# simochen/flowtrack.pytorch

Measured on AMD Instinct MI355X. Metric: pose crops/sec (ResNet-50 + 3-deconv head, 256x192), higher is better.
Workload: dtype fp16; 1 GPU; ResNet-50 pose head fp16, batch 64 x 256x192 synthetic crops per GPU (BASELINE.json configs[1]); per_gpu_batch=64, resident_batches=4, parallelism=dp1: batch sharded, one process per GPU

## Files before the change

flowtrack/pytorch_amd/csrc/conv_common.h:

```cpp
#pragma once
#include <stdlib.h>

#include <type_traits>

#include "ft_common.h"

#define FT_LDS_BARRIER() asm volatile("s_barrier" ::: "memory")

namespace ft {

struct ConvParams {
  const char* x;
  const char* w;
  const float* scale;
  const float* shift;
  const char* res;
  char* y;
  int M;
  int HqWq, Wq;
  int Hi, Wi;
  int sy;
  int x_cstride, x_coff;
  int kh, kw;
  int dmul;
// ... 229 lines not shown
        }
        return;
      }
      half_t* ybase = reinterpret_cast<half_t*>(p.y) + p.y_coff + co0;
      for (int idx = tid; idx < BP * NCH; idx += NT) {
        const int pl = idx / NCH, ch = idx % NCH;
        const long long o = s_opix[pl];
        if (o >= 0 && co0 + ch * 8 < p.Cout) {
          const uint4_t v = *reinterpret_cast<const uint4_t*>(s_tile + pl * ROWB + ((ch ^ (pl & (NCH - 1))) << 4));
          store_out16(ybase + o * p.y_cstride + ch * 8, v);
        }
      }
      return;
    }
  }

#pragma unroll
  for (int j = 0; j < MT_P; ++j) {
    const int m = m0 + wp * WT_P + j * 32 + l31;
    if (m >= p.M) continue;
    const int n = m / p.HqWq;
    const int rem = m - n * p.HqWq;
    const int qy = rem / p.Wq;
    const int qx = rem - qy * p.Wq;
    const int oy = qy * p.omul + py, ox = qx * p.omul + px;
    const size_t opix = ((size_t)n * p.Ho + oy) * p.Wo + ox;
#pragma unroll
    for (int i = 0; i < MT_C; ++i) {
#pragma unroll
      for (int rg = 0; rg < 4; ++rg) {
        const int cb = co0 + wc * WT_C + i * 32 + 8 * rg + 4 * lhi;
        if (cb >= p.Cout) continue;
        float v[4];
#pragma unroll
        for (int e = 0; e < 4; ++e) v[e] = acc[i][j][rg * 4 + e];
        if (p.scale) {
          const float4_t s = *reinterpret_cast<const float4_t*>(p.scale + cb);
#pragma unroll
          for (int e = 0; e < 4; ++e) v[e] *= s[e];
        }
        if (p.shift) {
          const float4_t s = *reinterpret_cast<const float4_t*>(p.shift + cb);
#pragma unroll
          for (int e = 0; e < 4; ++e) v[e] += s[e];
        }
        const bool full = cb + 3 < p.Cout;
        if (p.res) {
          const T* rp = reinterpret_cast<const T*>(p.res) + opix * p.res_cstride + p.res_coff + cb;
          if (full) {
            float r4[4];
            load4(rp, r4);
#pragma unroll
            for (int e = 0; e < 4; ++e) v[e] += r4[e];
          } else {
#pragma unroll
            for (int e = 0; e < 4; ++e)
              if (cb + e < p.Cout) v[e] += (float)rp[e];
          }
        }
#pragma unroll
        for (int e = 0; e < 4; ++e) v[e] = apply_act(v[e], p.act, p.slope);
        if (p.out_layout == FT_LAYOUT_NHWC) {
          T* yp = reinterpret_cast<T*>(p.y) + opix * p.y_cstride + p.y_coff + cb;
          if (full) {
            store4(yp, v);
          } else {
#pragma unroll
            for (int e = 0; e < 4; ++e)
              if (cb + e < p.Cout) yp[e] = (T)v[e];
          }
        } else {
          float* yp = reinterpret_cast<float*>(p.y);
          const size_t hw = (size_t)p.Ho * p.Wo;
          const size_t pix = (size_t)oy * p.Wo + ox;
#pragma unroll
          for (int e = 0; e < 4; ++e)
            if (cb + e < p.Cout) yp[((size_t)n * p.Cout + cb + e) * hw + pix] = v[e];
        }
      }
    }
  }
}

int launch_igemm8(const ConvParams& p, unsigned tiles, hipStream_t s);

}
```

flowtrack/pytorch_amd/csrc/conv_igemm.hip:

```cpp
#include <stdlib.h>

#include <type_traits>

#include "ft_common.h"

#ifndef FT_DMA_BKB
#define FT_DMA_BKB 64
#endif
#ifndef FT_DMA_STAGES
#define FT_DMA_STAGES 3
#endif
#include "conv_common.h"

namespace ft {

template <typename T, int BP, int BC, int WGP, int WGC, int BKB>
__global__ __launch_bounds__(256) void conv_igemm_kernel(const ConvParams p) {
  constexpr int VEC = Elem<T>::VEC;
  constexpr int CH = BKB / 16;
  constexpr int RPP = 256 / CH;
  constexpr int NB = BP / RPP;
  constexpr int NA = (BC + RPP - 1) / RPP;
  constexpr int WT_P = BP / WGP, WT_C = BC / WGC;
  constexpr int MT_P = WT_P / 32, MT_C = WT_C / 32;
// ... 2232 lines not shown
  p.h_ty = ceil_div(Hq, th);
  p.h_tx = ceil_div(Wq, tw);
  p.h_pw = tw + kq - 1;
  p.h_npix = (th + kq - 1) * p.h_pw;
  const int cch = d->transposed ? 64 : FT_HALO_CCH;
  p.h_npww = ceil_div(ceil_div(p.h_npix, 1024 / (cch * 2)), 4);
  if (p.h_npww > (d->transposed ? 5 : 6)) return FT_ERR_UNSUPPORTED;
  p.h_pb = p.h_npww * 4 * 1024;
  const int S = d->transposed ? 4 : 3;
  const size_t lds = (size_t)S * bc * 64 + 2 * (size_t)p.h_pb + 1024 + 128 * 8;
  const int N = p.M / p.HqWq;
  p.npt = N * p.h_ty * p.h_tx;
  p.nct = g.cout_pad / bc;
  if ((long long)p.npt * p.nct * p.nph > 0x7fffffffLL) return FT_ERR_UNSUPPORTED;
  dim3 grid(p.npt * p.nct * p.nph);
  int rc;
  if (d->transposed) {
    if (bc == 128) rc = tw == 16 ? launch_halo_k<128, 16, 4, 2, 4, 64>(p, grid, lds, s) : launch_halo_k<128, 8, 4, 2, 4, 64>(p, grid, lds, s);
    else rc = tw == 16 ? launch_halo_k<64, 16, 4, 2, 4, 64>(p, grid, lds, s) : launch_halo_k<64, 8, 4, 2, 4, 64>(p, grid, lds, s);
  } else {
    if (bc == 128) rc = tw == 16 ? launch_halo_k<128, 16, 9, 3, 3, FT_HALO_CCH>(p, grid, lds, s) : launch_halo_k<128, 8, 9, 3, 3, FT_HALO_CCH>(p, grid, lds, s);
    else rc = tw == 16 ? launch_halo_k<64, 16, 9, 3, 3, FT_HALO_CCH>(p, grid, lds, s) : launch_halo_k<64, 8, 9, 3, 3, FT_HALO_CCH>(p, grid, lds, s);
  }
  if (rc != FT_OK) return rc;
  FT_LAUNCH_CHECK("conv_halo_kernel");
  return FT_OK;
}

constexpr int kHintHalo = 1 << 30;

static bool stem_ok(const ft_conv_desc* d, const Geometry& g) {
  if (!g.rowpack || d->dtype != FT_F16 || d->has_residual || d->Cout != 64 || d->x_coff != 0) return false;
  if (!((d->kh == 7 && d->stride == 2) || (d->kh == 3 && d->stride == 1))) return false;
  const int runb = g.cin_pad * 2;
  if (!(runb == 64 || runb == 128 || (runb == 256 && d->kh == 7))) return false;
  if ((d->stride * d->x_cstride * 2) % 16 != 0 || d->pad - d->x_lpad > 0) return false;
  return d->out_layout == FT_LAYOUT_NHWC && d->y_coff % 8 == 0 && d->y_cstride % 8 == 0;
}

static bool halo_ok(const ft_conv_desc* d, const Geometry& g) {
  if (g.rowpack) return stem_ok(d, g);
  if (!g.dma || d->dtype != FT_F16 || d->has_residual) return false;
  if (!(d->transposed || (d->kh == 3 && d->kw == 3 && d->stride == 1 && d->pad == 1))) return false;
  return d->out_layout == FT_LAYOUT_NHWC && d->Cout % 8 == 0 && d->y_coff % 8 == 0 && d->y_cstride % 8 == 0;
}

static bool shift_n_ok(const ft_conv_desc* d, const Geometry& g) {
  if (d->shift_nstride < d->Cout || d->shift_nstride % 4 || d->pool || d->tail_cout > 0 || d->x2_cin > 0 || d->kh != 7 || d->stride != 2)
    return false;
  if (!stem_ok(d, g)) return false;
  if ((unsigned long long)d->N * d->Hi * d->x_wpitch * d->x_cstride * 2 >= (1ull << 31)) return false;
  int pw, npww, ntiles;
  size_t lds;
  return stem_persist_plan(d, g, &pw, &npww, &lds, &ntiles);
}

extern "C" int ft_conv_shift_nstride_supported(const ft_conv_desc* d) {
  Geometry g;
  const int st = geometry(d, &g);
  if (st != FT_OK) return st;
  return shift_n_ok(d, g) ? FT_OK : FT_ERR_UNSUPPORTED;
}

constexpr int kHintSkShift = 21;
__host__ __device__ constexpr int hint_sk(int code) { return code < 4 ? 1 << code : (code == 4 ? 3 : code + 0); }
constexpr int sk_code(int sk) { return sk == 1 ? 0 : sk == 2 ? 1 : sk == 4 ? 2 : sk == 8 ? 3 : sk == 3 ? 4 : sk; }

constexpr int kWide8 = 3;

static bool igemm8_ok(const ft_conv_desc* d, const Geometry& g) {
  if (!(g.dma && !g.rowpack && d->dtype == FT_F16 && g.kc2 == 0 && g.kc % 2 == 0 && g.cout_pad % 256 == 0 && g.nk / 2 >= 2)) return false;
  if (d->has_residual) return false;
  if ((unsigned long long)g.nphases * g.cout_pad * g.kpad * 2 >= (1ull << 31)) return false;
  if (g.cout_pad > 1024) return false;
  if (d->tail_cout > 0) return d->Cout == 256 && d->tail_cout <= 24;
  if (!(d->out_layout == FT_LAYOUT_NHWC && d->Cout % 8 == 0 && d->y_coff % 8 == 0 && d->y_cstride % 8 == 0)) return false;
  return (unsigned long long)d->N * d->Ho * d->Wo * d->y_cstride * 2 < (1ull << 31);
}

static bool tile_valid(const ft_conv_desc* d, const Geometry& g, int bp, int bc, int ks, int wide = 0, bool halo = false,
                       int sk = 1) {
  if (!g.dma) return false;
  if (wide == kWide8) {
    if (!igemm8_ok(d, g) || bp != 256 || bc != 256 || ks != 1 || halo) return false;
    if (sk != 1) {
      const int nk8 = g.nk / 2, per = (nk8 + sk - 1) / sk;
      if (sk < 2 || sk > 8 || d->tail_cout > 0 || per < 4 || nk8 - (sk - 1) * per < 2) return false;
    }
    return true;
  }
  if (sk != 1) {
    if (!(sk == 2 || sk == 4 || sk == 8) || ks != 1 || halo || g.kc2 > 0 || d->tail_cout > 0 || g.rowpack || bp > 128) return false;
    if ((g.nk >> wide) / sk < 4) return false;
  }
  if (g.kc2 > 0) {
    if (ks != 1 || halo) return false;
    if (wide && (g.kc2 % 2 != 0 || (g.kc >> 1) < 2)) return false;
  }
  if (halo) return halo_ok(d, g) && bp == 128 && (bc == 64 || (bc == 128 && !g.rowpack)) && g.cout_pad % bc == 0 && ks == 1 && wide == 0;
  if (wide < 0 || wide > 1) return false;
  if (wide && !(d->dtype == FT_F16 && g.kc % (1 << wide) == 0)) return false;
  if (wide && ks > 1) return false;
  if (bc == 256) {
    if (!(d->dtype == FT_F16 && (bp == 64 || bp == 128 || bp == 256) && ks == 1 && sk == 1 && g.cout_pad % 256 == 0)) return false;
    if (bp == 256 && wide != 1) return false;
    return true;
  }
  if (!((bp == 64 || bp == 128 || bp == 256) && (bc == 64 || bc == 128) && (ks == 1 || ks == 2 || ks == 4))) return false;
  if (g.cout_pad % bc != 0) return false;
  if (bp == 256 && !(bc == 128 && d->dtype == FT_F16 && ks == 1)) return false;
  if (ks > 1) {
    if (d->dtype != FT_F16 || (bp == 128 && bc == 64) || (ks == 4 && bp == 128)) return false;
    if ((g.nk >> wide) < 2 * ks) return false;
    if ((size_t)ks * kDmaStages * (bc + bp) * (kDmaBKB << wide) + 2048 + (size_t)bp * 8 > 160 * 1024) return false;
  }
  return true;
}

}

using namespace ft;

extern "C" int ft_conv_tile_candidates(const ft_conv_desc* d, int* hints, int max) {
  Geometry g;
  int st = geometry(d, &g);
  if (st != FT_OK) return -st;
  if (!hints || max <= 0) return -FT_ERR_INVALID_ARG;
  if (d->pool) return 0;
  if (d->tail_cout > 0) {
    if (max < 2 || d->Cout != 256 || !tile_valid(d, g, 256, 256, 1, kWide8)) return 0;
    hints[0] = 128 | (256 << 12) | (1 << 24);
    hints[1] = 256 | (256 << 12) | (1 << 24) | (kWide8 << kHintWideShift);
    return 2;
  }
  static const int kTiles[5][2] = {{256, 128}, {128, 128}, {128, 64}, {64, 128}, {64, 64}};
  int n = 0;
  for (const auto& t : kTiles)
    for (int ks = 1; ks <= 4; ks <<= 1)
      if (n < max && tile_valid(d, g, t[0], t[1], ks)) hints[n++] = t[0] | (t[1] << 12) | (ks << 24);
  for (const auto& t : kTiles)
    if (n < max && tile_valid(d, g, t[0], t[1], 1, 1)) hints[n++] = t[0] | (t[1] << 12) | (1 << 24) | (1 << kHintWideShift);
  for (int bp = 256; bp >= 64; bp >>= 1)
    for (int wide = 0; wide <= 1; ++wide)
      if (n < max && tile_valid(d, g, bp, 256, 1, wide)) hints[n++] = bp | (256 << 12) | (1 << 24) | (wide << kHintWideShift);
  if (n < max && tile_valid(d, g, 256, 256, 1, kWide8)) {
    hints[n++] = 256 | (256 << 12) | (1 << 24) | (kWide8 << kHintWideShift);
    const int Hq8 = d->transposed ? d->Hi : d->Ho, Wq8 = d->transposed ? d->Wi : d->Wo;
    const long long nblk8 = (long long)ceil_div(d->N * Hq8 * Wq8, 256) * (g.cout_pad / 256) * g.nphases;
    for (int lg = 1; lg <= 3; ++lg)
      if (n < max && nblk8 <= 160 && (nblk8 << lg) <= 640 && tile_valid(d, g, 256, 256, 1, kWide8, false, 1 << lg))
        hints[n++] = 256 | (256 << 12) | (1 << 24) | (kWide8 << kHintWideShift) | (lg << kHintSkShift);
    for (int sk = 3; sk <= 7; ++sk) {
      if (sk == 4) continue;
      if (n < max && nblk8 <= 160 && nblk8 * sk > 160 && nblk8 * sk <= 272 && tile_valid(d, g, 256, 256, 1, kWide8, false, sk))
        hints[n++] = 256 | (256 << 12) | (1 << 24) | (kWide8 << kHintWideShift) | (sk_code(sk) << kHintSkShift);
    }
  }
  {
    const int Hq = d->transposed ? d->Hi : d->Ho, Wq = d->transposed ? d->Wi : d->Wo;
    const long long M = (long long)d->N * Hq * Wq;
    static const int kSkTiles[3][2] = {{128, 128}, {64, 128}, {64, 64}};
    constexpr int sk_max_blocks = 256;
    for (const auto& t : kSkTiles) {
      if (g.cout_pad % t[1] != 0) continue;
      const long long nblk = (long long)ceil_div((int)M, t[0]) * (g.cout_pad / t[1]) * g.nphases;
      const int wide = tile_valid(d, g, t[0], t[1], 1, 1) ? 1 : 0;
      for (int lg = 1; lg <= 3; ++lg)
// ... 178 lines not shown
      const unsigned long long pb = (unsigned long long)d->N * d->Cin * d->Hi * d->Wi * 4;
      if (pb >= (1ull << 31)) return FT_ERR_UNSUPPORTED;
      p.x_bytes = (unsigned)pb;
    }
    return launch_stem_pool(p, d, g, s);
  }
  if (d->tail_cout > 0) {
    if (!g.dma || g.rowpack || x_bytes >= (1ull << 31) || g.cout_pad != d->Cout) return FT_ERR_UNSUPPORTED;
    if (!residual) return FT_ERR_INVALID_ARG;
    p.x_bytes = (unsigned)x_bytes;
    p.tail_w = static_cast<const char*>(residual);
    p.tail_cout = d->tail_cout;
    p.epi_lds = 1;
    const bool want8 = ((d->tile_hint >> kHintWideShift) & 3) == kWide8;
    if (want8 && d->Cout == 256 && tile_valid(d, g, 256, 256, 1, kWide8)) {
      p.npt = ceil_div(p.M, 256);
      p.nct = 1;
      p.kc = g.kc >> 1;
      p.nk = g.nk >> 1;
      if ((long long)p.npt * p.nph > 0x7fffffffLL) return FT_ERR_UNSUPPORTED;
      p.y_bytes = 0;
      p.w_bytes = (unsigned)((unsigned long long)g.nphases * g.cout_pad * g.kpad * 2);
      const int rc8 = launch_igemm8(p, (unsigned)(p.npt * p.nph), s);
      if (rc8 != FT_OK) return rc8;
      FT_LAUNCH_CHECK("conv_igemm8_kernel (tail)");
      return FT_OK;
    }
    p.npt = ceil_div(p.M, 128);
    p.nct = 1;
    if ((long long)p.npt * p.nph > 0x7fffffffLL) return FT_ERR_UNSUPPORTED;
    dim3 grid(p.npt * p.nph);
    const int rc = d->Cout == 256 ? launch_dma<half_t, 128, 256, 2, 4>(p, grid, s)
                   : d->Cout == 128 ? launch_dma<half_t, 128, 128, 2, 2>(p, grid, s) : launch_dma<half_t, 128, 64, 2, 2>(p, grid, s);
    if (rc != FT_OK) return rc;
    FT_LAUNCH_CHECK("conv_igemm_dma_kernel (tail)");
    return FT_OK;
  }
  if (g.dma && x_bytes < (1ull << 31)) {
    p.x_bytes = (unsigned)x_bytes;
    int bc = d->Cout % 128 == 0 ? 128 : 64;
    int bp = 128;
    auto blocks = [&](int bp_, int bc_) { return (long long)ceil_div(p.M, bp_) * (g.cout_pad / bc_) * g.nphases; };
    if (d->dtype == FT_F16 && bc == 128 && g.ntaps * g.cin_pad > 512 && blocks(256, 128) >= 2 * 256) bp = 256;
    if (blocks(bp, bc) < 384) bp = 64;
    if (blocks(bp, bc) < 384 && bc == 128) bc = 64;
    if (g.ntaps * g.cin_pad <= 512 && bc == 128) bp = 64;
    int ks = 1;
    if (d->dtype == FT_F16 && bp <= 128 && !(bp == 128 && bc == 64)) {
      const long long nblk = blocks(bp, bc);
      const long long per_cu = (nblk + 255) / 256;
      const size_t ring = (size_t)kDmaStages * (bc + bp) * kDmaBKB;
      for (int cand = 4; cand >= 2; cand >>= 1) {
        if (cand == 4 && bp == 128) continue;
        if (per_cu * (cand * ring + 2048) <= 160 * 1024 && per_cu * cand * 4 <= 32 && g.nk >= 8 * cand && nblk <= 768) {
          ks = cand;
          break;
        }
      }
    }
    int wide = 0, sk = 1;
    bool halo = false;
    if (d->dtype == FT_F16 && bp <= 128 && g.kc % 2 == 0 && g.ntaps * g.cin_pad >= 512 && blocks(bp, bc) <= 768) {
      wide = 1;
      ks = 1;
    }
    if (g.kc2 > 0) {
      ks = 1;
      if (wide && !tile_valid(d, g, bp, bc, 1, wide)) wide = 0;
    }
    const int hint = d->tile_hint;
    if (hint) {
      const int hbp = hint & 0xfff, hbc = (hint >> 12) & 0x1ff, hks = (hint >> 24) & 0xf;
      const int hwide = (hint >> kHintWideShift) & 3;
      const bool hhalo = (hint & kHintHalo) != 0;
      const int hsk = hint_sk((hint >> kHintSkShift) & 7);
      const int nbp = hbp ? hbp : bp, nbc = hbc ? hbc : bc, nks = hks ? hks : (hbp || hbc ? 1 : ks);
      if (tile_valid(d, g, nbp, nbc, nks, hwide, hhalo, hsk)) { bp = nbp; bc = nbc; ks = nks; wide = hwide; halo = hhalo; sk = hsk; }
    }
    if (sk > 1 && (!workspace || workspace_bytes < (size_t)sk * g.nphases * p.M * g.cout_pad * sizeof(float))) sk = 1;
    if (halo) return launch_halo(p, d, g, bc, s);
    if (wide == kWide8) {
      p.kc = g.kc >> 1;
      p.nk = g.nk >> 1;
      p.npt = ceil_div(p.M, 256);
      p.nct = g.cout_pad / 256;
      if ((long long)p.npt * p.nct * p.nph * sk > 0x7fffffffLL) return FT_ERR_UNSUPPORTED;
      p.y_bytes = (unsigned)((unsigned long long)d->N * d->Ho * d->Wo * d->y_cstride * 2);
      p.w_bytes = (unsigned)((unsigned long long)g.nphases * g.cout_pad * g.kpad * 2);
      if (sk > 1) {
        p.sk = sk;
        p.ws = static_cast<float*>(workspace);
      }
      const int rc8 = launch_igemm8(p, (unsigned)(p.npt * p.nct * p.nph * sk), s);
      if (rc8 != FT_OK) return rc8;
      FT_LAUNCH_CHECK("conv_igemm8_kernel");
      if (sk > 1) {
        const size_t total = (size_t)p.nph * p.M * (p.Cout_pad / 4);
        const unsigned rgrid = (unsigned)(total / 256 + 1 > 4096 ? 4096 : total / 256 + 1);
        hipLaunchKernelGGL(conv_splitk_reduce_kernel<half_t>, dim3(rgrid), dim3(256), 0, s, p);
        FT_LAUNCH_CHECK("conv_splitk_reduce_kernel");
      }
      return FT_OK;
    }
    if (wide) {
      p.kc = g.kc >> wide;
      p.kc2 = g.kc2 >> wide;
      p.nk = g.nk >> wide;
    }
    p.npt = ceil_div(p.M, bp);
    p.nct = g.cout_pad / bc;
    if ((long long)p.npt * p.nct * p.nph * sk > 0x7fffffffLL) return FT_ERR_UNSUPPORTED;
    dim3 grid(p.npt * p.nct * p.nph * sk);
    const char* const res_saved = p.res;
    if (sk > 1) {
      p.sk = sk;
      p.ws = static_cast<float*>(workspace);
      p.res = nullptr;
    }
    int rc;
    if (bc == 256) {
      if (wide == 1 && bp == 256) rc = launch_dma<half_t, 256, 256, 4, 2, 1, 128, 2>(p, grid, s);
      else if (wide == 1) rc = bp == 128 ? launch_dma<half_t, 128, 256, 2, 4, 1, 128, 2>(p, grid, s) : launch_dma<half_t, 64, 256, 1, 4, 1, 128, 2>(p, grid, s);
      else rc = bp == 128 ? launch_dma<half_t, 128, 256, 2, 4>(p, grid, s) : launch_dma<half_t, 64, 256, 1, 4>(p, grid, s);
    } else if (wide == 1) {
      if (bp == 256) rc = launch_dma<half_t, 256, 128, 4, 2, 1, 128, 2>(p, grid, s);
      else if (bp == 128 && bc == 128) rc = launch_dma<half_t, 128, 128, 2, 2, 1, 128, 2>(p, grid, s);
      else if (bp == 128) rc = launch_dma<half_t, 128, 64, 2, 2, 1, 128, 3>(p, grid, s);
      else if (bc == 128) rc = launch_dma<half_t, 64, 128, 2, 2, 1, 128, 3>(p, grid, s);
      else rc = launch_dma<half_t, 64, 64, 2, 2, 1, 128, 3>(p, grid, s);
    } else if (d->dtype == FT_F16) {
      if (bp == 256) rc = launch_dma<half_t, 256, 128, 4, 2>(p, grid, s);
      else if (bp == 128 && bc == 128)
        rc = ks == 2 ? launch_dma<half_t, 128, 128, 2, 2, 2>(p, grid, s) : launch_dma<half_t, 128, 128, 2, 2>(p, grid, s);
      else if (bp == 128) rc = launch_dma<half_t, 128, 64, 2, 2>(p, grid, s);
      else if (bc == 128)
        rc = ks == 4   ? launch_dma<half_t, 64, 128, 2, 2, 4>(p, grid, s)
             : ks == 2 ? launch_dma<half_t, 64, 128, 2, 2, 2>(p, grid, s)
                       : launch_dma<half_t, 64, 128, 2, 2>(p, grid, s);
      else
        rc = ks == 4   ? launch_dma<half_t, 64, 64, 2, 2, 4>(p, grid, s)
             : ks == 2 ? launch_dma<half_t, 64, 64, 2, 2, 2>(p, grid, s)
                       : launch_dma<half_t, 64, 64, 2, 2>(p, grid, s);
    } else {
      if (bp == 128 && bc == 128) rc = launch_dma<float, 128, 128, 2, 2>(p, grid, s);
      else if (bp == 128) rc = launch_dma<float, 128, 64, 2, 2>(p, grid, s);
      else if (bc == 128) rc = launch_dma<float, 64, 128, 2, 2>(p, grid, s);
      else rc = launch_dma<float, 64, 64, 2, 2>(p, grid, s);
    }
    if (rc != FT_OK) return rc;
    FT_LAUNCH_CHECK("conv_igemm_dma_kernel");
    if (sk > 1) {
      p.res = res_saved;
      const size_t total = (size_t)p.nph * p.M * (p.Cout_pad / 4);
      const unsigned rgrid = (unsigned)(total / 256 + 1 > 4096 ? 4096 : total / 256 + 1);
      if (d->dtype == FT_F16) hipLaunchKernelGGL(conv_splitk_reduce_kernel<half_t>, dim3(rgrid), dim3(256), 0, s, p);
      else hipLaunchKernelGGL(conv_splitk_reduce_kernel<float>, dim3(rgrid), dim3(256), 0, s, p);
      FT_LAUNCH_CHECK("conv_splitk_reduce_kernel");
    }
    return FT_OK;
  }
  if (g.dma) return FT_ERR_UNSUPPORTED;

  if (!d->transposed && d->Cout <= 2 && d->dtype == FT_F16 && d->kh == 3 && d->kw == 3 && d->stride == 1 &&
      d->pad == 1 && !d->has_residual && d->x_wpitch == 0 && d->x_cstride % 8 == 0 && d->x_coff % 8 == 0 && x_bytes < (1ull << 31)) {
    p.x_bytes = (unsigned)x_bytes;
    {
      const int nchunks = ceil_div(g.cin_groups, 4);
      const int ty = ceil_div(d->Ho, 12), tx = ceil_div(d->Wo, 16);
      const size_t lds = (size_t)4 * 16384 + (size_t)nchunks * 2048;
      if ((long long)d->N * ty * tx >= 256 && lds <= 160 * 1024 &&
          (long long)ty * 12 * tx * 16 * 100 <= (long long)d->Ho * d->Wo * 125) {
        p.h_ty = ty;
        p.h_tx = tx;
        p.npt = d->N * ty * tx;
        auto k = conv_pflow_mfma_kernel;
        if (lds > 64 * 1024) FT_RAISE_LDS(k, 160 * 1024);
// ... 58 lines not shown
```

flowtrack/pytorch_amd/csrc/conv_igemm8.hip:

```cpp
#include "conv_common.h"

namespace ft {

namespace {
constexpr int kT8 = 256;
constexpr int kRowB = 128;
constexpr int kHalfB = 128 * kRowB;
constexpr int kDbufB = 4 * kHalfB;
constexpr int kRingB = 2 * kDbufB;
}

namespace {
constexpr int kSlabB = 32 * 1024;
constexpr int kScaleOff = 24 * 1024, kShiftOff = 28 * 1024;
constexpr int kTailBiasOff = 2048;
constexpr int kMaxCout8 = 1024;
typedef uint32_t uint2v_t __attribute__((ext_vector_type(2)));
}
namespace {
__device__ __forceinline__ void ld2x16_asm(uint4_t& a, uint4_t& b, unsigned voff, const char* sbase) {
  asm volatile("global_load_dwordx4 %0, %2, %3\n\tglobal_load_dwordx4 %1, %2, %3 offset:1024"
               : "=&v"(a), "=&v"(b) : "v"(voff), "s"(sbase) : "memory");
}
template <int N>
// ... 381 lines not shown
    float4_t* slab = reinterpret_cast<float4_t*>(smem + kRingB);
    float16_t a2;
    auto send = [&](auto jc) __attribute__((always_inline)) {
      partial(jc, a2);
#pragma unroll
      for (int q4 = 0; q4 < 3; ++q4) {
        const float4_t v = {a2[4 * q4], a2[4 * q4 + 1], a2[4 * q4 + 2], a2[4 * q4 + 3]};
        slab[((wp * 2 + (1 - wc)) * 3 + q4) * 64 + lane] = v;
      }
    };
    if (wc == 0) { send(I1{}); partial(I0{}, a2); } else { send(I0{}); partial(I1{}, a2); }
    asm volatile("s_waitcnt lgkmcnt(0)" ::: "memory");
    FT_LDS_BARRIER();
    if (!(p.dbg & 4)) {
      const long long hw = (long long)p.Ho * p.Wo;
      int n, pix;
      if (out_pixel(m0, py, px, wc, l31, n, pix)) {
#pragma unroll
        for (int q4 = 0; q4 < 3; ++q4) {
          const float4_t o = slab[((wp * 2 + wc) * 3 + q4) * 64 + lane];
          const float4_t bq = *reinterpret_cast<const float4_t*>(smem + kRingB + kShiftOff + kTailBiasOff + (8 * q4 + 4 * lhi) * 4);
#pragma unroll
          for (int e = 0; e < 4; ++e) {
            const int co2 = e + 8 * q4 + 4 * lhi;
            if (co2 < p.tail_cout) {
              const float v = a2[4 * q4 + e] + o[e] + bq[e];
              if (p.out_layout == FT_LAYOUT_NHWC)
                reinterpret_cast<half_t*>(p.y)[((long long)n * hw + pix) * p.y_cstride + p.y_coff + co2] = (half_t)v;
              else
                reinterpret_cast<float*>(p.y)[((long long)n * p.tail_cout + co2) * hw + pix] = v;
            }
          }
        }
      }
    }
  };

  int o_m0, o_co0, o_phase, o_ksplit, o_nkt;
  int n_m0 = 0, n_co0 = 0, n_phase = 0, n_ksplit = 0, n_nkt = 0;
  setup(local, o_m0, o_co0, o_phase, o_ksplit, o_nkt);
  prologue();
  asm volatile("s_waitcnt vmcnt(6)" ::: "memory");
  FT_LDS_BARRIER();
  if (wc == 1) FT_LDS_BARRIER();
#pragma unroll
  for (int i = 0; i < 4; ++i)
#pragma unroll
    for (int j = 0; j < 2; ++j)
#pragma unroll
      for (int r = 0; r < 16; ++r) acc[i][j][r] = 0.f;
  int t_rem = o_nkt;
  bool more = false;
  for (;;) {
    if (t_rem == 2) {
      local += x_slots;
      more = local < x_count;
      if (more) setup(local, n_m0, n_co0, n_phase, n_ksplit, n_nkt);
      else kill();
      asm volatile("s_waitcnt lgkmcnt(0)" ::: "memory");
    }
    ktile();
    if (--t_rem == 0) {
      if (wc == 0) FT_LDS_BARRIER();
      if constexpr (MODE == 1) epilogue_tail(o_m0, o_phase);
      else if constexpr (MODE == 2) epilogue_partial(o_m0, o_co0, o_phase, o_ksplit);
      else epilogue_store(o_m0, o_co0, o_phase);
      if (!more) break;
      o_m0 = n_m0; o_co0 = n_co0; o_phase = n_phase; o_ksplit = n_ksplit; o_nkt = n_nkt;
      t_rem = o_nkt;
      __builtin_amdgcn_sched_barrier(0);
      if (wc == 1) FT_LDS_BARRIER();
#pragma unroll
      for (int i = 0; i < 4; ++i)
#pragma unroll
        for (int j = 0; j < 2; ++j)
#pragma unroll
          for (int r = 0; r < 16; ++r) acc[i][j][r] = 0.f;
      asm volatile("s_waitcnt lgkmcnt(0)" ::: "memory");
    }
  }
#endif
}

int launch_igemm8(const ConvParams& p, unsigned tiles, hipStream_t s) {
  constexpr size_t lds = (size_t)kRingB + (size_t)kSlabB;
  static int cus[64] = {};
  int dev = 0;
  FT_HIP_CHECK(hipGetDevice(&dev));
  if (dev < 0 || dev >= 64) return FT_ERR_INVALID_ARG;
  if (!cus[dev]) {
    int n = 0;
    FT_HIP_CHECK(hipDeviceGetAttribute(&n, hipDeviceAttributeMultiprocessorCount, dev));
    cus[dev] = n > 0 ? n : 256;
  }
  const unsigned grid = tiles < (unsigned)cus[dev] ? tiles : (unsigned)cus[dev];
  if (p.tail_w) {
    FT_RAISE_LDS(conv_igemm8_kernel<1>, lds);
    hipLaunchKernelGGL(conv_igemm8_kernel<1>, dim3(grid), dim3(512), lds, s, p);
  } else if (p.sk > 1) {
    FT_RAISE_LDS(conv_igemm8_kernel<2>, lds);
    hipLaunchKernelGGL(conv_igemm8_kernel<2>, dim3(grid), dim3(512), lds, s, p);
  } else {
    FT_RAISE_LDS(conv_igemm8_kernel<0>, lds);
    hipLaunchKernelGGL(conv_igemm8_kernel<0>, dim3(grid), dim3(512), lds, s, p);
  }
  return FT_OK;
}

}
```

Before: 59500 crops/s.

## Add 192-pixel tile variant of the wide8 persistent igemm conv kernel

Adds a new persistent igemm8 kernel that uses a 192-pixel by 256-channel tile (3 pixel sub-blocks per wave pair) instead of 256x256. The tile validator and launcher now accept bp=192, and tile counts are computed from bp. The goal is to improve tile quantization and load balance across CUs for conv shapes whose M does not divide well by 256. In exchange it lowers per-tile reuse and adds a large new hand-scheduled kernel. The fused tail mode is unsupported for this variant.

```diff
diff --git a/flowtrack/pytorch_amd/csrc/conv_common.h b/flowtrack/pytorch_amd/csrc/conv_common.h
--- a/flowtrack/pytorch_amd/csrc/conv_common.h
+++ b/flowtrack/pytorch_amd/csrc/conv_common.h
@@ -335,6 +335,6 @@
   }
 }
 
-int launch_igemm8(const ConvParams& p, unsigned tiles, hipStream_t s);
-
-}
+int launch_igemm8(const ConvParams& p, unsigned tiles, hipStream_t s, int bp = 256);
+
+}
diff --git a/flowtrack/pytorch_amd/csrc/conv_igemm.hip b/flowtrack/pytorch_amd/csrc/conv_igemm.hip
--- a/flowtrack/pytorch_amd/csrc/conv_igemm.hip
+++ b/flowtrack/pytorch_amd/csrc/conv_igemm.hip
@@ -2338,7 +2338,8 @@
                        int sk = 1) {
   if (!g.dma) return false;
   if (wide == kWide8) {
-    if (!igemm8_ok(d, g) || bp != 256 || bc != 256 || ks != 1 || halo) return false;
+    if (!igemm8_ok(d, g) || (bp != 256 && bp != 192) || bc != 256 || ks != 1 || halo) return false;
+    if (bp == 192 && d->tail_cout > 0) return false;
     if (sk != 1) {
       const int nk8 = g.nk / 2, per = (nk8 + sk - 1) / sk;
       if (sk < 2 || sk > 8 || d->tail_cout > 0 || per < 4 || nk8 - (sk - 1) * per < 2) return false;
@@ -2683,7 +2684,7 @@
     if (wide == kWide8) {
       p.kc = g.kc >> 1;
       p.nk = g.nk >> 1;
-      p.npt = ceil_div(p.M, 256);
+      p.npt = ceil_div(p.M, bp);
       p.nct = g.cout_pad / 256;
       if ((long long)p.npt * p.nct * p.nph * sk > 0x7fffffffLL) return FT_ERR_UNSUPPORTED;
       p.y_bytes = (unsigned)((unsigned long long)d->N * d->Ho * d->Wo * d->y_cstride * 2);
@@ -2692,7 +2693,7 @@
         p.sk = sk;
         p.ws = static_cast<float*>(workspace);
       }
-      const int rc8 = launch_igemm8(p, (unsigned)(p.npt * p.nct * p.nph * sk), s);
+      const int rc8 = launch_igemm8(p, (unsigned)(p.npt * p.nct * p.nph * sk), s, bp);
       if (rc8 != FT_OK) return rc8;
       FT_LAUNCH_CHECK("conv_igemm8_kernel");
       if (sk > 1) {
diff --git a/flowtrack/pytorch_amd/csrc/conv_igemm8.hip b/flowtrack/pytorch_amd/csrc/conv_igemm8.hip
--- a/flowtrack/pytorch_amd/csrc/conv_igemm8.hip
+++ b/flowtrack/pytorch_amd/csrc/conv_igemm8.hip
@@ -487,7 +487,354 @@
 #endif
 }
 
-int launch_igemm8(const ConvParams& p, unsigned tiles, hipStream_t s) {
+namespace {
+constexpr int kP8 = 192;
+[[maybe_unused]] constexpr int kPartB = 64 * kRowB;
+}
+
+template <int MODE>
+__global__ __launch_bounds__(512, 2) void conv_igemm8_p192_kernel(const ConvParams p) {
+  static_assert(MODE == 0 || MODE == 2, "the fused tail keeps the 256-pixel tile");
+#if defined(__HIP_DEVICE_COMPILE__)
+  extern __shared__ __attribute__((aligned(16))) char smem[];
+  typedef __attribute__((address_space(3))) void* lds_ptr;
+  constexpr unsigned kOOB = 0x80000000u;
+  using I0 = std::integral_constant<int, 0>;
+  using I1 = std::integral_constant<int, 1>;
+  using I2 = std::integral_constant<int, 2>;
+
+  const int tid = threadIdx.x;
+  const int lane = tid & 63;
+  const int wave = __builtin_amdgcn_readfirstlane(tid >> 6);
+  const int wq = wave & 3, wh = wave >> 2;
+  const int l31 = lane & 31, lhi = lane >> 5;
+
+  const int tiles = p.npt * p.nct * p.nph;
+  const int total = tiles * p.sk;
+  const int xcd = blockIdx.x & 7;
+  int local = blockIdx.x >> 3;
+  int x_start, x_count, x_slots;
+  {
+    const int q = total >> 3, r = total & 7;
+    x_start = xcd < r ? xcd * (q + 1) : r * (q + 1) + (xcd - r) * q;
+    x_count = q + (xcd < r ? 1 : 0);
+    x_slots = ((int)gridDim.x - xcd + 7) >> 3;
+  }
+  if (local >= x_count) return;
+
+  const __amdgpu_buffer_rsrc_t rsrc_x = __builtin_amdgcn_make_buffer_rsrc(const_cast<char*>(p.x), 0, p.x_bytes, 0x00020000);
+  const __amdgpu_buffer_rsrc_t rsrc_w = __builtin_amdgcn_make_buffer_rsrc(const_cast<char*>(p.w), 0, p.w_bytes, 0x00020000);
+  const int krow = p.Kpad * 2;
+  const int cstride_b = p.x_cstride * 2;
+  const int nk_sk = (p.nk + p.sk - 1) / p.sk;
+
+  const int lrow = lane >> 3, pos = lane & 7;
+  const int lc16 = (pos ^ (((wave & 1) << 2) | (lrow >> 1))) << 4;
+  const unsigned w_voff = (p.dbg & 256) ? kOOB : (unsigned)(((wave >> 2) * 64 + (wave & 3) * 8 + lrow) * krow + lc16);
+
+  {
+    float* const ls = reinterpret_cast<float*>(smem + kRingB + kScaleOff);
+    float* const lh = reinterpret_cast<float*>(smem + kRingB + kShiftOff);
+    for (int c = tid; c < p.Cout_pad; c += 512) {
+      ls[c] = p.scale ? p.scale[c] : 1.f;
+      lh[c] = p.shift ? p.shift[c] : 0.f;
+    }
+    __syncthreads();
+  }
+
+  int s_woff = 0;
+  int b_base[3];
+  unsigned b_yx[3];
+  unsigned cur_voff[3];
+  int kt_hi = 0, s_kt = 0, s_cc = 0, s_ky = 0, s_kx = 0;
+  unsigned p2_voff = kOOB;
+  int p2_cc = 0;
+  auto refresh = [&]() __attribute__((always_inline)) {
+    const bool live = s_kt < kt_hi;
+    const int dy = p.dmul * s_ky, dx = p.dmul * s_kx;
+    const int delta = (dy * p.Wi + dx) * cstride_b;
+#pragma unroll
+    for (int j = 0; j < 3; ++j) {
+      const int iy = (int)(b_yx[j] & 0xffffu) - 0x4000 + dy, ix = (int)(b_yx[j] >> 16) - 0x4000 + dx;
+      const bool ok = live && (unsigned)iy < (unsigned)p.Hi && (unsigned)ix < (unsigned)p.Wi;
+      cur_voff[j] = ok ? (unsigned)(b_base[j] + delta) : kOOB;
+    }
+  };
+  auto setup = [&](int loc, int& m0, int& co0, int& phase, int& ksplit, int& nkt) __attribute__((always_inline)) {
+    int logical = x_start + loc;
+    ksplit = logical / tiles;
+    logical -= ksplit * tiles;
+    const int ctile = logical % p.nct;
+    const int t = logical / p.nct;
+    phase = t % p.nph;
+    m0 = (t / p.nph) * kP8;
+    co0 = ctile * kT8;
+    const int py = phase >> 1, px = phase & 1;
+    const int dbase_y = p.transposed ? py : -p.pad;
+    const int dbase_x = p.transposed ? px : -p.pad_x;
+    const int kt_lo = ksplit * nk_sk;
+    kt_hi = kt_lo + nk_sk < p.nk ? kt_lo + nk_sk : p.nk;
+    nkt = kt_hi > kt_lo ? kt_hi - kt_lo : 0;
+    s_woff = (phase * p.Cout_pad + co0) * krow;
+#pragma unroll
+    for (int j = 0; j < 3; ++j) {
+      const int m = m0 + (wave >> 2) * 96 + j * 32 + (wave & 3) * 8 + lrow;
+      unsigned yx = 0xffffffffu;
+      int base = 0;
+      if (m < p.M && !(p.dbg & 64)) {
+        const int n = m / p.HqWq;
+        const int rem = m - n * p.HqWq;
+        const int qy = rem / p.Wq;
+        const int qx = rem - qy * p.Wq;
+        const int iy0 = qy * p.sy + dbase_y, ix0 = qx * p.sy + dbase_x;
+        base = ((n * p.Hi + iy0) * p.Wi + ix0) * cstride_b + p.x_coff * 2 + lc16;
+        yx = (unsigned)(iy0 + 0x4000) | ((unsigned)(ix0 + 0x4000) << 16);
+      }
+      b_base[j] = base;
+      b_yx[j] = yx;
+    }
+    s_kt = kt_lo;
+    const int tap0 = kt_lo / p.kc;
+    s_cc = kt_lo - tap0 * p.kc;
+    s_ky = tap0 / p.kw;
+    s_kx = tap0 - s_ky * p.kw;
+    refresh();
+  };
+  auto kill = [&]() __attribute__((always_inline)) {
+    kt_hi = s_kt = 0;
+#pragma unroll
+    for (int j = 0; j < 3; ++j) cur_voff[j] = kOOB;
+  };
+  auto advance = [&]() __attribute__((always_inline)) {
+    p2_voff = cur_voff[2];
+    p2_cc = s_cc;
+    ++s_kt;
+    if (++s_cc == p.kc) {
+      s_cc = 0;
+      if (++s_kx == p.kw) { s_kx = 0; ++s_ky; }
+      refresh();
+    }
+  };
+  auto stage_w = [&](int dofs, int kt) __attribute__((always_inline)) {
+    const unsigned v = kt < kt_hi ? w_voff : kOOB;
+#pragma unroll
+    for (int h = 0; h < 2; ++h)
+#pragma unroll
+      for (int u = 0; u < 2; ++u)
+        __builtin_amdgcn_raw_ptr_buffer_load_lds(rsrc_w, (lds_ptr)(smem + dofs + h * kHalfB + u * kPartB + wave * 1024), 16, v,
+                                                 s_woff + kt * kRowB + (u * 128 + h * 32) * krow, 0, 0);
+  };
+  auto stage_p = [&](int dofs, auto jc, unsigned voff, int cc) __attribute__((always_inline)) {
+    constexpr int j = decltype(jc)::value;
+    __builtin_amdgcn_raw_ptr_buffer_load_lds(rsrc_x, (lds_ptr)(smem + dofs + 2 * kHalfB + j * kPartB + wave * 1024), 16, voff,
+                                             cc * kRowB, 0, 0);
+  };
+  auto prologue = [&]() __attribute__((always_inline)) {
+    stage_p(0, I0{}, cur_voff[0], s_cc);
+    stage_w(0, s_kt);
+    stage_p(0, I1{}, cur_voff[1], s_cc);
+    stage_p(0, I2{}, cur_voff[2], s_cc);
+    advance();
+    stage_p(kDbufB, I0{}, cur_voff[0], s_cc);
+    stage_w(kDbufB, s_kt);
+    stage_p(kDbufB, I1{}, cur_voff[1], s_cc);
+    advance();
+  };
+
+  const int fkey = ((lhi ^ ((l31 >> 1) & 7)) << 4);
+  int rd_p[4], rd_w[4];
+#pragma unroll
+  for (int kk = 0; kk < 4; ++kk) {
+    rd_p[kk] = (2 * kHalfB + (wh * 32 + l31) * kRowB + fkey) ^ (kk << 5);
+    rd_w[kk] = ((wq * 32 + l31) * kRowB + fkey) ^ (kk << 5);
+  }
+  int dofs = 0;
+
+  float16_t acc[2][3];
+  uint4_t wf[2][4], pf[3][4];
+
+#define FT8_MFMA(i, j, W, P)                                                                                          \
+  acc[i][j] = __builtin_amdgcn_mfma_f32_32x32x16_f16(__builtin_bit_cast(half8_t, W), __builtin_bit_cast(half8_t, P), \
+                                                     acc[i][j], 0, 0, 0)
+
+  auto ktile = [&]() __attribute__((always_inline)) {
+#pragma unroll
+    for (int kk = 0; kk < 4; ++kk) pf[0][kk] = *reinterpret_cast<const uint4_t*>(smem + rd_p[kk]);
+    __builtin_amdgcn_sched_barrier(0);
+#pragma unroll
+    for (int ii = 0; ii < 2; ++ii)
+#pragma unroll
+      for (int kk = 0; kk < 4; ++kk) wf[ii][kk] = *reinterpret_cast<const uint4_t*>(smem + rd_w[kk] + ii * kHalfB);
+    __builtin_amdgcn_sched_barrier(0);
+    stage_p(dofs ^ kDbufB, I2{}, p2_voff, p2_cc);
+    asm volatile("s_waitcnt lgkmcnt(8)" ::: "memory");
+    FT_LDS_BARRIER();
+    asm volatile("s_waitcnt lgkmcnt(0)" ::: "memory");
+    __builtin_amdgcn_sched_barrier(0);
+    __builtin_amdgcn_s_setprio(1);
+#pragma unroll
+    for (int kk = 0; kk < 4; ++kk) {
+      FT8_MFMA(0, 0, wf[0][kk], pf[0][kk]);
+      FT8_MFMA(1, 0, wf[1][kk], pf[0][kk]);
+    }
+    __builtin_amdgcn_s_setprio(0);
+    __builtin_amdgcn_sched_barrier(0);
+    FT_LDS_BARRIER();
+#pragma unroll
+    for (int kk = 0; kk < 4; ++kk) pf[1][kk] = *reinterpret_cast<const uint4_t*>(smem + rd_p[kk] + kPartB);
+    __builtin_amdgcn_sched_barrier(0);
+    stage_p(dofs, I0{}, cur_voff[0], s_cc);
+    asm volatile("s_waitcnt lgkmcnt(0)" ::: "memory");
+    FT_LDS_BARRIER();
+    __builtin_amdgcn_sched_barrier(0);
+    __builtin_amdgcn_s_setprio(1);
+#pragma unroll
+    for (int kk = 0; kk < 4; ++kk) {
+      FT8_MFMA(0, 1, wf[0][kk], pf[1][kk]);
+      FT8_MFMA(1, 1, wf[1][kk], pf[1][kk]);
+    }
+    __builtin_amdgcn_s_setprio(0);
+    __builtin_amdgcn_sched_barrier(0);
+    FT_LDS_BARRIER();
+#pragma unroll
+    for (int kk = 0; kk < 4; ++kk) pf[2][kk] = *reinterpret_cast<const uint4_t*>(smem + rd_p[kk] + 2 * kPartB);
+    __builtin_amdgcn_sched_barrier(0);
+    stage_w(dofs, s_kt);
+    stage_p(dofs, I1{}, cur_voff[1], s_cc);
+    advance();
+#pragma unroll
+    for (int kk = 0; kk < 4; ++kk) { rd_p[kk] ^= kDbufB; rd_w[kk] ^= kDbufB; }
+    dofs ^= kDbufB;
+    asm volatile("s_waitcnt vmcnt(6) lgkmcnt(0)" ::: "memory");
+    FT_LDS_BARRIER();
+    __builtin_amdgcn_sched_barrier(0);
+    __builtin_amdgcn_s_setprio(1);
+#pragma unroll
+    for (int kk = 0; kk < 4; ++kk) {
+      FT8_MFMA(0, 2, wf[0][kk], pf[2][kk]);
+      FT8_MFMA(1, 2, wf[1][kk], pf[2][kk]);
+    }
+    __builtin_amdgcn_s_setprio(0);
+    __builtin_amdgcn_sched_barrier(0);
+    FT_LDS_BARRIER();
+  };
+#undef FT8_MFMA
+
+  const __amdgpu_buffer_rsrc_t rsrc_y = __builtin_amdgcn_make_buffer_rsrc(p.y, 0, p.y_bytes, 0x00020000);
+  const float act_s = p.act == FT_ACT_RELU ? 0.f : (p.act == FT_ACT_LEAKY ? p.slope : 1.f);
+  auto act1 = [&](float v) __attribute__((always_inline)) { return __builtin_fmaf(act_s, __builtin_fminf(v, 0.f), __builtin_fmaxf(v, 0.f)); };
+  auto activated = [&](int i, int j, int rg, int cb) __attribute__((always_inline)) -> uint2v_t {
+    const float4_t sc = *reinterpret_cast<const float4_t*>(smem + kRingB + kScaleOff + cb * 4);
+    const float4_t sh = *reinterpret_cast<const float4_t*>(smem + kRingB + kShiftOff + cb * 4);
+    float v[4];
+#pragma unroll
+    for (int e = 0; e < 4; ++e) v[e] = act1(acc[i][j][rg * 4 + e] * sc[e] + sh[e]);
+    const half4_t h = {(half_t)v[0], (half_t)v[1], (half_t)v[2], (half_t)v[3]};
+    return __builtin_bit_cast(uint2v_t, h);
+  };
+  auto epilogue_store = [&](int m0, int co0, int phase) __attribute__((always_inline)) {
+    const int py = phase >> 1, px = phase & 1;
+    char* const tb = smem + kRingB + wave * 2048;
+    const int rrow = lane >> 2, rpos = lane & 3;
+#pragma unroll
+    for (int j = 0; j < 3; ++j) {
+      unsigned vrow[2];
+#pragma unroll
+      for (int ps = 0; ps < 2; ++ps) {
+        const int row = ps * 16 + rrow;
+        const int m = m0 + wh * 96 + j * 32 + row;
+        unsigned v = kOOB;
+        if (m < p.M) {
+          const int n = m / p.HqWq;
+          const int rem = m - n * p.HqWq;
+          const int qy = rem / p.Wq;
+          const int qx = rem - qy * p.Wq;
+          const int pix = (n * p.Ho + qy * p.omul + py) * p.Wo + (qx * p.omul + px);
+          v = (unsigned)((pix * p.y_cstride + p.y_coff + co0 + wq * 64 + ((rpos ^ ((row >> 1) & 3)) << 3)) * 2);
+        }
+        vrow[ps] = v;
+      }
+#pragma unroll
+      for (int i = 0; i < 2; ++i) {
+#pragma unroll
+        for (int rg = 0; rg < 4; ++rg) {
+          const uint2v_t h = activated(i, j, rg, co0 + wq * 64 + i * 32 + 8 * rg + 4 * lhi);
+          *reinterpret_cast<uint2v_t*>(tb + l31 * 64 + ((rg ^ ((l31 >> 1) & 3)) << 4) + lhi * 8) = h;
+        }
+#pragma unroll
+        for (int ps = 0; ps < 2; ++ps) {
+          const int row = ps * 16 + rrow;
+          const uint4_t o = *reinterpret_cast<const uint4_t*>(tb + row * 64 + rpos * 16);
+          const int cchunk = co0 + wq * 64 + i * 32 + ((rpos ^ ((row >> 1) & 3)) << 3);
+          const unsigned v = (cchunk < p.Cout && !(p.dbg & 4)) ? vrow[ps] + i * 64 : kOOB;
+          __builtin_amdgcn_raw_buffer_store_b128(o, rsrc_y, v, 0, FT8_STORE_AUX);
+        }
+      }
+    }
+  };
+  auto epilogue_partial = [&](int m0, int co0, int phase, int ksplit) __attribute__((always_inline)) {
+    float* wsb = p.ws + ((size_t)ksplit * p.nph + phase) * (size_t)p.M * p.Cout_pad;
+#pragma unroll
+    for (int j = 0; j < 3; ++j) {
+      const int m = m0 + wh * 96 + j * 32 + l31;
+      if (m >= p.M || (p.dbg & 4)) continue;
+#pragma unroll
+      for (int i = 0; i < 2; ++i)
+#pragma unroll
+        for (int rg = 0; rg < 4; ++rg) {
+          const int cb = co0 + wq * 64 + i * 32 + 8 * rg + 4 * lhi;
+          const float4_t v = {acc[i][j][rg * 4], acc[i][j][rg * 4 + 1], acc[i][j][rg * 4 + 2], acc[i][j][rg * 4 + 3]};
+          *reinterpret_cast<float4_t*>(wsb + (size_t)m * p.Cout_pad + cb) = v;
+        }
+    }
+  };
+
+  int o_m0, o_co0, o_phase, o_ksplit, o_nkt;
+  int n_m0 = 0, n_co0 = 0, n_phase = 0, n_ksplit = 0, n_nkt = 0;
+  setup(local, o_m0, o_co0, o_phase, o_ksplit, o_nkt);
+  prologue();
+  asm volatile("s_waitcnt vmcnt(6)" ::: "memory");
+  FT_LDS_BARRIER();
+  if (wh == 1) FT_LDS_BARRIER();
+#pragma unroll
+  for (int i = 0; i < 2; ++i)
+#pragma unroll
+    for (int j = 0; j < 3; ++j)
+#pragma unroll
+      for (int r = 0; r < 16; ++r) acc[i][j][r] = 0.f;
+  int t_rem = o_nkt;
+  bool more = false;
+  for (;;) {
+    if (t_rem == 2) {
+      local += x_slots;
+      more = local < x_count;
+      if (more) setup(local, n_m0, n_co0, n_phase, n_ksplit, n_nkt);
+      else kill();
+      asm volatile("s_waitcnt lgkmcnt(0)" ::: "memory");
+    }
+    ktile();
+    if (--t_rem == 0) {
+      if (wh == 0) FT_LDS_BARRIER();
+      if constexpr (MODE == 2) epilogue_partial(o_m0, o_co0, o_phase, o_ksplit);
+      else epilogue_store(o_m0, o_co0, o_phase);
+      if (!more) break;
+      o_m0 = n_m0; o_co0 = n_co0; o_phase = n_phase; o_ksplit = n_ksplit; o_nkt = n_nkt;
+      t_rem = o_nkt;
+      __builtin_amdgcn_sched_barrier(0);
+      if (wh == 1) FT_LDS_BARRIER();
+#pragma unroll
+      for (int i = 0; i < 2; ++i)
+#pragma unroll
+        for (int j = 0; j < 3; ++j)
+#pragma unroll
+          for (int r = 0; r < 16; ++r) acc[i][j][r] = 0.f;
+      asm volatile("s_waitcnt lgkmcnt(0)" ::: "memory");
+    }
+  }
+#endif
+}
+
+int launch_igemm8(const ConvParams& p, unsigned tiles, hipStream_t s, int bp) {
   constexpr size_t lds = (size_t)kRingB + (size_t)kSlabB;
   static int cus[64] = {};
   int dev = 0;
@@ -499,7 +846,16 @@
     cus[dev] = n > 0 ? n : 256;
   }
   const unsigned grid = tiles < (unsigned)cus[dev] ? tiles : (unsigned)cus[dev];
-  if (p.tail_w) {
+  if (bp == kP8) {
+    if (p.tail_w) return FT_ERR_UNSUPPORTED;
+    if (p.sk > 1) {
+      FT_RAISE_LDS(conv_igemm8_p192_kernel<2>, lds);
+      hipLaunchKernelGGL(conv_igemm8_p192_kernel<2>, dim3(grid), dim3(512), lds, s, p);
+    } else {
+      FT_RAISE_LDS(conv_igemm8_p192_kernel<0>, lds);
+      hipLaunchKernelGGL(conv_igemm8_p192_kernel<0>, dim3(grid), dim3(512), lds, s, p);
+    }
+  } else if (p.tail_w) {
     FT_RAISE_LDS(conv_igemm8_kernel<1>, lds);
     hipLaunchKernelGGL(conv_igemm8_kernel<1>, dim3(grid), dim3(512), lds, s, p);
   } else if (p.sk > 1) {
```

Result: slower. 58110 crops/s (-2.3%).
